# Villen-Lab/pyAscore

Hardware: AMD Instinct MI355X
Metric: PSMs/sec (Ascore.score) at 1/2/4/8 MI355X + HBM-roofline % (higher is better)
Workload: dtype f32/f64 scalar + i32 counts

## Files before the change

pyascore_amd/csrc/fused_core.hip.h:

```cpp
#ifndef PYA_FUSED_CORE_H
#define PYA_FUSED_CORE_H
#include "score_core.hip.h"
#include "localize_core.hip.h"

#define FUSED_ROUND 3

struct FusedLds {
    uint16_t *grid;
    uint4 *cum_lut;
    PeakEntry *peaks;
    float2 *resd;
    uint8_t *rkl;
    uint32_t *rec;
    float *wsl;
    float *mass_l;
    uint32_t *flag_l;
    uint8_t *site_pos;
    float *selm;
    unsigned char *sort_raw;
    PushedEntry *pushed;
    unsigned long long *site_alt;
    uint32_t *site_max, *site_tie, *n_pushed;
    float *sc;
    uint32_t *c_tr, *c_cnt;
    uint32_t *bad_tasks;
    uint32_t *t_lo, *t_off;
    float *srt_v;
    uint8_t *srt_h;
    int32_t *c_depth;
    uint32_t *c_site;
};

__host__ __device__ static inline size_t fused_align16(size_t v) { return (v + 15) & ~(size_t)15; }
__host__ __device__ static inline size_t fused_sort_bytes(uint32_t n) {
    if (n <= 64) return ((size_t)n * 10 + 15) & ~(size_t)15;
    return (((size_t)n * 6 + 15) & ~(size_t)15) + ((size_t)n / 64 + 2) * 16 + 2 * 128 * 2;
}
__host__ __device__ static inline uint32_t fused_site_cap(uint32_t push_cap) {
    const uint32_t v = (push_cap + 3u) & ~3u;
    return v > 64u ? 64u : (v < 4u ? 4u : v);
}
__host__ __device__ static inline size_t fused_post_bytes(uint32_t n_cap, uint32_t push_cap, uint32_t ent_cap, uint32_t ndir,
                                                          bool multi_z) {
    return fused_align16(fused_sort_bytes(n_cap)) + (size_t)push_cap * 16 + (size_t)fused_site_cap(push_cap) * 16 + 16 +
           (size_t)(1 + FUSED_ROUND) * 40 + (size_t)FUSED_ROUND * (16 * ndir + 4 + 4) + 16 + 64 +
           (multi_z ? fused_align16((size_t)FUSED_ROUND * ndir * 2 * ent_cap * 4) +
                          fused_align16((size_t)FUSED_ROUND * ndir * 2 * ent_cap)
                    : 0);
}
__host__ __device__ static inline size_t fused_walk_bytes(uint32_t cap) {
    return 16 * 16 + ((size_t)cap + PYA_TABLE_PAD) * 8;
}
__host__ __device__ static inline size_t fused_kept_bytes(uint32_t n_cap, uint32_t stride, uint32_t pos_cap, uint32_t ent_cap,
                                                          uint32_t ndir) {
    return fused_align16(((size_t)pos_cap + 1) * 8) + fused_align16((size_t)ent_cap * stride) + (size_t)n_cap * 16 + 256 +
           fused_align16((size_t)pos_cap + 1) + (size_t)(1 + FUSED_ROUND) * ndir * ent_cap * 4;
}
__host__ __device__ static inline size_t fused_lds_bytes(uint32_t cap, uint32_t n_cap, uint32_t stride, uint32_t pos_cap,
                                                         uint32_t ent_cap, uint32_t push_cap, uint32_t ndir, bool multi_z) {
    const size_t walk = fused_walk_bytes(cap), post = fused_post_bytes(n_cap, push_cap, ent_cap, ndir, multi_z);
    return PYA_GRID_CELLS * 2 + fused_align16(walk > post ? walk : post) +
           fused_kept_bytes(n_cap, stride, pos_cap, ent_cap, ndir) + 16;
}

DEV FusedLds fused_carve(unsigned char *raw, uint32_t cap, uint32_t n_cap, uint32_t stride, uint32_t pos_cap,
                         uint32_t ent_cap, uint32_t push_cap, uint32_t ndir, bool multi_z) {
    FusedLds f;
    f.grid = (uint16_t *)raw;
    size_t o = PYA_GRID_CELLS * 2;
    f.cum_lut = (uint4 *)(raw + o);
    f.peaks = (PeakEntry *)(raw + o + 16 * 16);
    f.sort_raw = raw + o;
    size_t q = o + fused_align16(fused_sort_bytes(n_cap));
    f.pushed = (PushedEntry *)(raw + q);
    q += (size_t)push_cap * sizeof(PushedEntry);
    const size_t sc = fused_site_cap(push_cap);
    f.site_alt = (unsigned long long *)(raw + q);
    q += sc * 8;
    f.site_max = (uint32_t *)(raw + q);
    q += sc * 4;
    f.site_tie = (uint32_t *)(raw + q);
    q += sc * 4;
    f.n_pushed = (uint32_t *)(raw + q);
    q += 16;
    f.sc = (float *)(raw + q);
    q += (size_t)(1 + FUSED_ROUND) * 40;
    f.c_tr = (uint32_t *)(raw + q);
    q += (size_t)FUSED_ROUND * ndir * 8;
    f.c_cnt = (uint32_t *)(raw + q);
    q += (size_t)FUSED_ROUND * ndir * 8;
    f.c_depth = (int32_t *)(raw + q);
    q += FUSED_ROUND * 4;
    f.c_site = (uint32_t *)(raw + q);
    q += FUSED_ROUND * 4;
    f.bad_tasks = (uint32_t *)(raw + q);
    q += 16;
    f.t_lo = (uint32_t *)(raw + q);
    f.t_off = f.t_lo + 8;
    q += 64;
    f.srt_v = (float *)(raw + q);
    q += fused_align16((size_t)FUSED_ROUND * ndir * 2 * ent_cap * 4);
    f.srt_h = (uint8_t *)(raw + q);
    const size_t walk = fused_walk_bytes(cap), post = fused_post_bytes(n_cap, push_cap, ent_cap, ndir, multi_z);
    o += fused_align16(walk > post ? walk : post);
    f.resd = (float2 *)(raw + o);
    o += fused_align16(((size_t)pos_cap + 1) * 8);
    f.rkl = (uint8_t *)(raw + o);
    o += fused_align16((size_t)ent_cap * stride);
    f.rec = (uint32_t *)(raw + o);
    o += (size_t)n_cap * 12;
    f.wsl = (float *)(raw + o);
    o += (size_t)n_cap * 4;
    f.mass_l = (float *)(raw + o);
    f.flag_l = (uint32_t *)(raw + o + 128);
    f.site_pos = (uint8_t *)(raw + o + 256);
    f.selm = (float *)(raw + o + 256 + fused_align16((size_t)pos_cap + 1));
    return f;
}


template <bool BZ>
DEV void walk_record_steps(const float2 *&rp, int rstride, StepBits &bits, float &running, const uint4 *lut, CumCounts &cum,
                           const PeakTable &tab, int zmax, double A, double B, uint8_t *&ro, int stride, int count) {
    for (int i = 0; i < count; i++, rp += rstride) {
        const float2 mm = *rp;
        running = (bits.next() ? mm.y : mm.x) + running;
        const double m = BZ ? (double)running + A : ((double)running + A) - B;
        for (int z = 1; z <= zmax; z++, ro += stride) {
            const Look k = look4(tab, charge_mz(m, z));
            int rk = k.best;
            if (k.more()) rk = look_rest(tab, k);
            cum.add(lut[rk]);
            *ro = (uint8_t)rk;
        }
    }
}
DEV CumCounts walk_record(const float2 *resd, const uint4 *lut, const PeakTable &tab, int L, int zmax, uint64_t resmask, int dir,
                          double A, double B, bool all_b_zero, uint8_t *rkl, int stride, int w) {
    const uint64_t tmask = dir ? (__brevll(resmask) >> (64 - L)) : resmask;
    const float2 *rp = resd + (dir ? L - 1 : 0);
    const int rstride = dir ? -1 : 1;
    uint8_t *ro = rkl + w;
    float running = 0.f;
    CumCounts cum = {0u, 0u, 0u};
    if (tab.half_check) {
        const uint32_t tlo = (uint32_t)tmask, thi = (uint32_t)(tmask >> 32);
        for (int step = 0; step + 1 < L; step++, rp += rstride) {
            const float2 mm = *rp;
            const uint32_t word = step < 32 ? tlo : thi;
            const bool mod = (word >> (step & 31)) & 1u;
            running = (mod ? mm.y : mm.x) + running;
            const double m = ((double)running + A) - B;
            for (int z = 1; z <= zmax; z++, ro += stride) {
                const int rk = match_rank_lds(tab, charge_mz(m, z));
                cum.add(lut[rk]);
                *ro = (uint8_t)rk;
            }
        }
        return cum;
    }
    const uint64_t M = msb_first_from(tmask, 0);
    const int n = L - 1;
    for (int seg = 0; seg < 2; seg++) {
        StepBits bits = {seg ? (uint32_t)M : (uint32_t)(M >> 32)};
        int c = (n < seg * 32 + 32 ? n : seg * 32 + 32) - seg * 32;
        if (c < 0) c = 0;
        if (all_b_zero) walk_record_steps<true>(rp, rstride, bits, running, lut, cum, tab, zmax, A, B, ro, stride, c);
        else walk_record_steps<false>(rp, rstride, bits, running, lut, cum, tab, zmax, A, B, ro, stride, c);
    }
    return cum;
}

DEV void walk_mz_only(const float2 *resd, int L, int zmax, uint64_t resmask, int dir, double A, double B, float *out) {
    const uint64_t tmask = dir ? (__brevll(resmask) >> (64 - L)) : resmask;
    const uint64_t M = msb_first_from(tmask, 0);
    const float2 *rp = resd + (dir ? L - 1 : 0);
    const int rstride = dir ? -1 : 1;
    const int Lm1 = L - 1;
    float running = 0.f;
    int step = 0;
    for (int seg = 0; seg < 2; seg++) {
        StepBits bits = {seg ? (uint32_t)M : (uint32_t)(M >> 32)};
        const int end = Lm1 < seg * 32 + 32 ? Lm1 : seg * 32 + 32;
        for (; step < end; step++, rp += rstride) {
            const float2 mm = *rp;
            running = (bits.next() ? mm.y : mm.x) + running;
            const double m = ((double)running + A) - B;
            out[step] = (float)(m + 1.007825);
            for (int z = 2; z <= zmax; z++) out[(z - 1) * Lm1 + step] = charge_mz(m, z);
        }
    }
}

DEV void walk_sums_only(const float2 *resd, int L, uint64_t resmask, int dir, float *out) {
    const uint64_t tmask = dir ? (__brevll(resmask) >> (64 - L)) : resmask;
    const uint64_t M = msb_first_from(tmask, 0);
    const float2 *rp = resd + (dir ? L - 1 : 0);
    const int rstride = dir ? -1 : 1;
    const int Lm1 = L - 1;
    float running = 0.f;
    int step = 0;
    for (int seg = 0; seg < 2; seg++) {
        StepBits bits = {seg ? (uint32_t)M : (uint32_t)(M >> 32)};
        const int end = Lm1 < seg * 32 + 32 ? Lm1 : seg * 32 + 32;
        for (; step < end; step++, rp += rstride) {
            const float2 mm = *rp;
            running = (bits.next() ? mm.y : mm.x) + running;
            out[step] = running;
        }
    }
}

DEV int partners_in_run(const float *run, int n, int p2, float me, int side, float err) {
    int j = 0;
    for (int step = p2 >> 1; step > 0; step >>= 1) {
        const int probe = j + step;
        const float o = probe - 1 < n ? run[probe - 1] : __builtin_huge_valf();
        const float dd = side ? (o - me) : (me - o);
        if (side ? (dd <= -err) : (dd >= err)) j = probe;
    }
    int cnt = 0;
    for (int q = j; q < j + 2 && q < n; q++) {
        const float dd = side ? (run[q] - me) : (me - run[q]);
        cnt += (__builtin_fabsf(dd) < err) ? 1 : 0;
    }
    return cnt;
}

#define FUSED_LOCAL_CHUNKS 8
struct LocalTable {
    const float *mz;
    const uint8_t *rank;
    int R, status;
};

template <bool BOTH, bool ZM, bool WIDE = false>
DEV bool fused_body(const BatchDev &b, uint32_t psm, unsigned char *lds_raw, uint32_t cap, uint32_t n_cap, uint32_t stride,
                    uint32_t pos_cap, uint32_t ent_cap, uint32_t push_cap, const LocalTable *local = nullptr) {
    const int lane = lane_id();
    const DevConfig *cfg = b.cfg;
    const int ndir = BOTH ? 2 : 1;
    const FusedLds f = fused_carve(lds_raw, cap, n_cap, stride, pos_cap, ent_cap, push_cap, (uint32_t)ndir, ZM);
    STAMP_BEGIN();
    STAMP_T(b, 38, false);
    float lmz[FUSED_LOCAL_CHUNKS];
    uint32_t lrk[FUSED_LOCAL_CHUNKS];
    if (local) {
#pragma unroll
        for (int q = 0; q < FUSED_LOCAL_CHUNKS; q++) {
            const int i = q * 64 + lane_id();
            lmz[q] = i < local->R ? local->mz[i] : __builtin_huge_valf();
            lrk[q] = i < local->R ? (uint32_t)local->rank[i] : (uint32_t)PYA_NO_MATCH;
        }
        wave_lds_sync();
    }
    if (lane < 32) {
        f.mass_l[lane] = cfg->res_mass[lane];
        f.flag_l[lane] = cfg->res_modifiable[lane];
    }
    const uint64_t *dw = b.desc + (size_t)psm * PYA_DESC_WORDS;
    const int64_t p0 = (int64_t)dw[0], pep0 = (int64_t)dw[1], s0 = (int64_t)dw[2], a0 = (int64_t)dw[3];
    const uint64_t w4 = dw[4], w5 = dw[5];
    const int L = (int)(w4 & 0xffffu), n_aux = (int)((w4 >> 16) & 0xffffu), k = (int)((w4 >> 32) & 0xffffu);
    const int zmax = ZM ? (int)(w4 >> 56) : 1;
    const int N = (int)(uint32_t)w5;
    const uint64_t *order = b.order_tab + (uint32_t)(w5 >> 32);
    const int status = local ? local->status : b.status[psm];
    const int R = local ? local->R : (int)b.ret_n[psm];

    const uint32_t max_k = b.max_k;
    float *out_asc = b.ascores + (size_t)psm * max_k;
    uint64_t *out_alt = b.alt_mask + (size_t)psm * max_k;
    for (uint32_t a = lane; a < max_k; a += 64) {
        out_asc[a] = 0.f;
        out_alt[a] = 0ull;
    }
    if (status != PYA_ST_OK) {
        if (lane == 0) {
            b.best_score[psm] = -1.f;
            b.best_sig[psm] = 0ull;
            b.n_sig_out[psm] = -1;
        }
        return false;
    }
    STAMP_T(b, 39, false);
    const bool two_pass = BOTH && WIDE && N > 32;
    const int s = (BOTH && !two_pass) ? (lane & 31) : lane;
    const int dir = BOTH ? (two_pass ? 0 : (lane >> 5)) : (cfg->n_fwd > 0 ? 0 : 1);
    const bool active = s < N;
    const uint32_t letter = lane < L ? (uint32_t)b.pep[pep0 + lane] : (uint32_t)'A';
    const uint64_t bits = active ? order[s] : 0ull;
    uint32_t aux_pos = 0;
    float aux_mass = 0.f;
    if (lane < n_aux) {
        aux_pos = b.aux_pos[a0 + lane];
        aux_mass = b.aux_mass[a0 + lane];
    }
    if (local) {
#pragma unroll
        for (int q = 0; q < FUSED_LOCAL_CHUNKS; q++) {
            const int i = q * 64 + lane;
            if (i < R + PYA_TABLE_PAD) {
                PeakEntry e;
                e.mz = lmz[q];
                e.rank = lrk[q];
                f.peaks[i] = e;
            }
        }
    } else {
        copy_peak_table(b.ret + p0, R, f.peaks, lane, 64);
    }
    PeakTable tab;
    tab.e = f.peaks;
    tab.g_cell = nullptr;
    tab.g_e = b.ret + p0;
    tab.n = R;
    tab.err = cfg->mz_error;
    tab.half_check = cfg->mz_error > 0.49f;
    double Af = 0., Bf = 0., Ab = 0., Bb = 0.;
    if (cfg->n_fwd > 0) type_constants(cfg->types[0], &Af, &Bf);
    if (cfg->n_fwd < cfg->n_types) type_constants(cfg->types[cfg->n_fwd], &Ab, &Bb);
    wave_lds_sync();
    STAMP_T(b, 48, false);
    float m0, m1;
    uint64_t site_mask;
    {
        const bool in = lane < L;
        const uint32_t li = (letter - 'A') & 31u;
        m0 = f.mass_l[li];
        const bool modifiable = in && ((f.flag_l[li] & 1u) || (cfg->allow_n && lane == 0) || (cfg->allow_c && lane == L - 1));
        m1 = m0 + cfg->mod_mass;
        for (int base = 0; base < n_aux; base += 64) {
            const int n = n_aux - base < 64 ? n_aux - base : 64;
            if (base > 0) {
                aux_pos = 0;
                aux_mass = 0.f;
                if (lane < n) {
                    aux_pos = b.aux_pos[a0 + base + lane];
                    aux_mass = b.aux_mass[a0 + base + lane];
                }
            }
            for (int j = 0; j < n; j++) {
                const uint32_t pos = (uint32_t)__builtin_amdgcn_readlane((int)aux_pos, j);
                const float am = __int_as_float(__builtin_amdgcn_readlane(__float_as_int(aux_mass), j));
                const int idx = pos > 0 ? (int)pos - 1 : 0;
                if (idx == lane) {
                    m0 += am;
                    m1 += am;
                }
            }
        }
        site_mask = __ballot(modifiable);
        if (in) f.resd[lane] = make_float2(m0, m1);
        if (modifiable) f.site_pos[mask_rank(site_mask)] = (uint8_t)lane;
    }
    STAMP_T(b, 49, false);
    grid_build(&tab, f.grid);
    STAMP_T(b, 50, false);
    if (lane < 16) f.cum_lut[lane] = fused_cum_entry((uint32_t)lane);
    const int Lm1 = L - 1;
    const uint64_t resmask = deposit_sites(bits, site_mask);
    const int w = !active ? (int)stride - 1 : (BOTH ? dir * N + s : s);
    const bool presorted = !__any(lane < L && !(m0 > 0.f && m1 > 0.f));
    const float wide_min = 2.f * cfg->mz_error + 0.02f;
    const bool wide = !__any(lane < L && !(m0 > wide_min && m1 > wide_min));
    wave_lds_sync();
    STAMP_T(b, 40, false);
    CumCounts cum = walk_record(f.resd, f.cum_lut, tab, L, zmax, resmask, dir, dir ? Ab : Af, dir ? Bb : Bf, Bf == 0. && Bb == 0.,
                                f.rkl, (int)stride, w);
    if (two_pass) {
        const CumCounts back = walk_record(f.resd, f.cum_lut, tab, L, zmax, resmask, 1, Ab, Bb, Bf == 0. && Bb == 0., f.rkl, (int)stride,
                                           active ? N + s : (int)stride - 1);
        cum.a += back.a;
        cum.b += back.b;
        cum.c += back.c;
    } else if (BOTH) {
        uint32_t *r3 = f.rec + (size_t)s * 3;
        if (active && lane >= 32) {
            r3[0] = cum.a;
            r3[1] = cum.b;
            r3[2] = cum.c;
        }
        wave_lds_sync();
        if (active && lane < 32) {
            cum.a += r3[0];
            cum.b += r3[1];
            cum.c += r3[2];
        }
    }
    wave_lds_sync();
    STAMP_T(b, 41, false);

    const uint32_t nfrag = (uint32_t)ndir * (uint32_t)Lm1 * (uint32_t)zmax;
    int fail = 0;
    float ws = 0.f;
// ... 437 lines not shown
```

pyascore_amd/csrc/host_internal.h:

```cpp
#ifndef PYA_HOST_INTERNAL_H
#define PYA_HOST_INTERNAL_H
#include <hip/hip_runtime_api.h>

#include <algorithm>
#include <atomic>
#include <cmath>
#include <cstdarg>
#include <cstddef>
#include <cstdio>
#include <cstdlib>
#include <chrono>
#include <cstring>
#include <condition_variable>
#include <map>
#include <memory>
#include <mutex>
#include <string>
#include <thread>
#include <unordered_map>
#include <vector>

#include "../../include/pyascore_hip.h"
#include "common.h"

void pya_score_table_extend(float mz_error, uint32_t n_top, uint32_t n_to, std::vector<float> &lut,
                            std::vector<uint32_t> &off);
extern "C" {
size_t pya_bin_lds_bytes(uint32_t cap);
size_t pya_score_lds_bytes(uint32_t cap, uint32_t prefix, uint32_t with_nl, uint32_t compact);
size_t pya_localize_lds_bytes(uint32_t push_cap, uint32_t n_cap, uint32_t pos_cap, uint32_t pool_cap, uint32_t sb);
int pya_launch_bin(const BatchDev *b, const uint32_t *d_ids, uint32_t n_ids, uint32_t cap, uint32_t types, hipStream_t stream);
int pya_launch_bin_select(const BatchDev *b, const uint32_t *d_ids, uint32_t n_ids, uint32_t scap, uint32_t types, hipStream_t stream);
size_t pya_bin_select_lds_bytes(uint32_t scap);
int pya_launch_bin_exact(const BatchDev *b, uint32_t n_total, uint32_t cap, uint32_t types, hipStream_t stream);
int pya_launch_fan_out(const uint32_t *d_spec_of, const uint32_t *d_spec_ret_n, const int32_t *d_spec_status, uint32_t *d_ret_n,
                       int32_t *d_status, uint32_t n_psm, hipStream_t stream);
int pya_launch_score(const BatchDev *b, const uint32_t *d_ids, uint32_t n_ids, uint32_t cap, uint32_t prefix,
                     uint32_t with_nl, uint32_t compact, uint32_t node_cap, uint32_t node_cols, uint32_t node_words,
                     uint32_t res_cap, uint32_t nl_cap, hipStream_t stream);
size_t pya_score_node_lds_bytes(uint32_t cap, uint32_t with_nl, uint32_t node_cap, uint32_t node_cols, uint32_t node_words,
                                uint32_t res_cap, uint32_t nl_cap);
int pya_launch_localize(const BatchDev *b, const uint32_t *d_ids, uint32_t n_ids, uint32_t push_cap,
                        uint32_t n_cap, uint32_t pos_cap, uint32_t pool_cap, uint32_t sb, uint32_t gtp,
                        uint32_t plain, uint32_t sort_room, hipStream_t stream);
size_t pya_tiny_lds_bytes(uint32_t cap, uint32_t prefix, uint32_t with_nl, uint32_t compact, uint32_t push_cap,
                          uint32_t n_cap, uint32_t pos_cap, uint32_t pool_cap, uint32_t sb);
int pya_launch_tiny(const BatchDev *b, uint32_t n_psm, uint32_t cap, uint32_t prefix, uint32_t with_nl,
                    uint32_t compact, uint32_t push_cap, uint32_t n_cap, uint32_t pos_cap, uint32_t pool_cap,
                    uint32_t sb, uint32_t gtp, hipStream_t stream);
size_t pya_one_lds_bytes(uint32_t cap, uint32_t prefix, uint32_t with_nl, uint32_t compact, uint32_t push_cap, uint32_t n_cap,
                         uint32_t pos_cap, uint32_t pool_cap, uint32_t sb, uint32_t use_fused, uint32_t f_n_cap, uint32_t f_stride,
                         uint32_t f_ent_cap, uint32_t f_push_cap, uint32_t multi_z);
int pya_launch_one(const BatchDev *b, const OneMeta *m, uint32_t cap, uint32_t prefix, uint32_t with_nl, uint32_t compact,
                   uint32_t push_cap, uint32_t n_cap, uint32_t pos_cap, uint32_t pool_cap, uint32_t sb, uint32_t gtp,
                   uint32_t use_fused, uint32_t f_n_cap, uint32_t f_stride, uint32_t f_ent_cap, uint32_t f_push_cap,
                   uint32_t multi_z, int32_t *host_status, uint32_t *host_flag, hipStream_t stream);
int pya_launch_ambiguity(const BatchDev *b, uint32_t psm, uint32_t peak_cap, uint32_t list_cap,
                         uint64_t ref_bits, uint64_t oth_bits, const float *d_scores, float ref_ws,
                         float oth_ws, float *d_out, hipStream_t stream);
int pya_launch_debug_sort(const float *d_keys, uint32_t n, uint32_t *d_perm, hipStream_t stream);
int pya_launch_pack_records(const float *best_score, const int32_t *n_sig, const uint64_t *best_sig, const float *ascores,
                            const uint64_t *alt_mask, uint32_t k, uint32_t res_k, uint64_t n_psm, int32_t *out, hipStream_t stream);
int pya_launch_debug_wave_ops(const int32_t *d_in, int32_t *d_out, hipStream_t stream);
size_t pya_score_big_lds_bytes(uint32_t cap, uint32_t pos_cap, uint32_t kc);
int pya_launch_score_big(const BatchDev *b, const uint32_t *d_ids, uint32_t n_ids, uint32_t cap, uint32_t pos_cap, uint32_t kc,
                         uint32_t inline_on, hipStream_t stream);
size_t pya_localize_recount_lds_bytes(uint32_t cap, uint32_t push_cap, uint32_t pos_cap, uint32_t pool_cap, uint32_t sb);
size_t pya_localize_hash_lds_bytes(uint32_t push_cap, uint32_t n_cap, uint32_t pos_cap, uint32_t sb, uint32_t vc, uint32_t hs,
                                   uint32_t pp, uint32_t max_k, uint32_t n_nl);
int pya_launch_localize_hash(const BatchDev *b, const uint32_t *d_ids, uint32_t n_ids, uint32_t push_cap, uint32_t n_cap,
                             uint32_t pos_cap, uint32_t pool_cap, uint32_t sb, uint32_t gtp, uint32_t vc, uint32_t hs, uint32_t pp,
                             uint32_t n_nl, hipStream_t stream);
int pya_launch_localize_recount(const BatchDev *b, const uint32_t *d_ids, uint32_t n_ids, uint32_t cap, uint32_t push_cap,
                                uint32_t pos_cap, uint32_t pool_cap, uint32_t sb, uint32_t gtp, uint32_t *d_redo_count, uint32_t *d_redo_ids, hipStream_t stream);
int pya_launch_score_big_list(const BatchDev *b, const uint32_t *d_count, const uint32_t *d_ids, uint32_t n_max, uint32_t cap,
                              uint32_t pos_cap, uint32_t kc, hipStream_t stream);
uint32_t pya_big_inline_max(void);
size_t pya_fused_lds_bytes(uint32_t cap, uint32_t n_cap, uint32_t stride, uint32_t pos_cap, uint32_t ent_cap, uint32_t push_cap,
                           uint32_t both, uint32_t multi_z);
int pya_launch_fused(const BatchDev *b, const uint32_t *d_ids, uint32_t n_ids, uint32_t cap, uint32_t n_cap,
                     uint32_t stride, uint32_t pos_cap, uint32_t ent_cap, uint32_t push_cap, uint32_t both,
                     uint32_t multi_z, uint32_t *d_redo_count, uint32_t *d_redo_ids, hipStream_t stream);
size_t pya_score_cnt_lds_bytes(uint32_t cap, uint32_t pos_cap, uint32_t kc, uint32_t k_cap, uint32_t n_cap);
int pya_launch_score_cnt(const BatchDev *b, const uint32_t *d_ids, uint32_t n_ids, uint32_t cap, uint32_t pos_cap, uint32_t kc, uint32_t k_cap,
                         uint32_t n_cap, hipStream_t stream);
size_t pya_score_cntg_lds_bytes(uint32_t cap, uint32_t pos_cap, uint32_t k_cap, uint32_t n_cap, uint32_t nl_cap);
int pya_launch_score_cntg(const BatchDev *b, const uint32_t *d_ids, uint32_t n_ids, uint32_t cap, uint32_t pos_cap, uint32_t k_cap, uint32_t n_cap,
                          uint32_t nl_cap, hipStream_t stream);
size_t pya_bin_global_scratch_bytes(uint32_t cap);
int pya_launch_bin_global(const BatchDev *b, const uint32_t *d_ids, uint32_t n_ids, unsigned char *d_scratch, uint64_t stride,
                          uint32_t cap, uint32_t types, hipStream_t stream);
size_t pya_general_lds_bytes(uint32_t l_cap, uint32_t list_cap);
size_t pya_general_scratch_bytes(uint32_t n_cap, uint32_t push_cap);
int pya_launch_general(const BatchDev *b, const uint32_t *d_ids, uint32_t n_ids, unsigned char *d_scratch, const uint64_t *d_scratch_off,
                       uint32_t l_cap, uint32_t list_cap, hipStream_t stream);
int pya_launch_general_ambiguity(const BatchDev *b, uint32_t psm, uint32_t l_cap, uint32_t list_cap, uint64_t ref_bits,
                                 uint64_t oth_bits, const float *d_scores, uint32_t n_scores, float ref_ws, float oth_ws,
                                 float *d_out, hipStream_t stream);
size_t pya_evidence_lds_bytes(uint32_t l_cap, uint32_t list_cap);
int pya_launch_evidence(const BatchDev *b, const uint32_t *d_ids, uint32_t n_ids, void *d_out, uint32_t l_cap, uint32_t list_cap,
                        hipStream_t stream);
size_t pya_ions_lds_bytes(uint32_t l_cap, uint32_t list_cap);
uint32_t pya_ions_scan_tiles(uint32_t n);
int pya_launch_ions(const BatchDev *b, const uint32_t *d_ids, uint32_t n_ids, const void *d_evid, int64_t *d_off, void *d_out, uint64_t cap,
                    uint32_t *d_over, uint32_t l_cap, uint32_t list_cap, hipStream_t stream);
int pya_launch_ions_scan(int64_t *d_off, uint32_t n, uint64_t *d_tiles, hipStream_t stream);
size_t pya_named_lds_bytes(uint32_t l_cap, uint32_t list_cap);
int pya_launch_named(const BatchDev *b, const uint32_t *d_ids, uint32_t n_ids, const int64_t *d_q_off, const uint64_t *d_q_bits,
                     uint64_t n_q, void *d_out, int32_t *d_counts, float *d_scores, uint32_t *d_over, uint32_t l_cap,
                     uint32_t list_cap, hipStream_t stream);
size_t pya_sites_lds_bytes(uint32_t l_cap, uint32_t list_cap);
int pya_launch_sites(const BatchDev *b, const uint32_t *d_ids, uint32_t n_ids, const int64_t *d_site_off, uint64_t n_out,
                     uint32_t sig_cap, void *d_out, uint32_t l_cap, hipStream_t stream);
size_t pya_probs_lds_bytes(uint32_t l_cap, const PcCaps *caps, uint32_t sw);
size_t pya_probs_cnt_bytes(const PcCaps *caps);
int pya_launch_probs(const BatchDev *b, const uint32_t *d_ids, uint32_t n_ids, const int64_t *d_site_off, uint64_t n_out,
                     uint32_t sig_cap, void *d_out, void *d_psms, uint32_t l_cap, const PcCaps *caps, uint32_t sw, hipStream_t stream);
size_t pya_ranked_lds_bytes(uint32_t l_cap, const PcCaps *caps, uint32_t sw);
int pya_launch_ranked(const BatchDev *b, const uint32_t *d_ids, uint32_t n_ids, const int64_t *d_site_off, uint32_t top_k,
                      uint32_t sig_cap, void *d_out, uint32_t l_cap, const PcCaps *caps, uint32_t sw, hipStream_t stream);
int pya_launch_rollup_clear(void *d_table, uint64_t n_slots, hipStream_t stream);
int pya_launch_rollup(const int64_t *d_site_off, uint64_t n_psm, uint64_t n_rec, const void *d_site_probs, const void *d_psm_probs,
                      const int32_t *d_slot, uint64_t n_slots, double threshold, const uint32_t *d_psm_id, uint32_t psm_base,
                      const uint64_t *best_sig, const float *ascores, uint32_t max_k, void *d_table, uint32_t *d_over, uint32_t grid[2],
                      hipStream_t stream);
size_t pya_mz_profile_lds_bytes(uint32_t l_cap);
int pya_launch_mz_profile(const BatchDev *b, const uint32_t *d_ids, uint32_t n_ids, const int32_t *d_run, uint64_t n_slots,
                          const pya_mz_profile_params *prm, void *d_table, uint32_t *d_over, uint32_t l_cap, hipStream_t stream);
int pya_launch_mz_fit(const void *d_table, uint64_t n_slots, double inv_ppm, uint32_t min_ions, void *d_cal, hipStream_t stream);
int pya_launch_mz_apply(const void *d_mz, uint32_t mz_type, const int64_t *d_peak_off, uint64_t n_spectra, const int32_t *d_run,
                        const void *d_cal, uint64_t n_slots, double inv_band, void *d_out, uint32_t *d_over, hipStream_t stream);
uint64_t pya_flr_layout_bytes(uint64_t n_slots);
int pya_launch_flr(const void *d_table, uint64_t n_slots, const uint8_t *d_cls, uint32_t reported_only, void *d_work, void *d_out,
                   uint32_t *d_order, uint32_t *d_n_ranked, hipEvent_t *phase, hipStream_t stream);
uint64_t pya_pform_layout_bytes(uint64_t n_entries);
int pya_launch_pform(const int64_t *d_site_off, uint64_t n_psm, const void *d_site_probs, const void *d_psm_probs, const int32_t *d_group,
                     double threshold, const uint32_t *d_psm_id, uint32_t psm_base, const uint64_t *best_sig, const float *ascores, uint32_t max_k,
                     const void *d_src0, uint64_t n0, const void *d_src1, uint64_t n1, void *d_work, void *d_out, uint64_t cap, uint32_t *d_n,
                     hipEvent_t *phase, hipStream_t stream);
int pya_launch_localize_redo(const BatchDev *b, const uint32_t *d_count, const uint32_t *d_ids, uint32_t n_max,
                             uint32_t push_cap, uint32_t n_cap, uint32_t pos_cap, uint32_t pool_cap, uint32_t sb,
                             uint32_t gtp, hipStream_t stream);
}



const size_t kMaxLds = 160 * 1024;
const uint32_t kBucketLimits[] = {64, 512, 4096, PYA_FAST_SIGNATURES};
const int kNumBuckets = 4;
const size_t kRedoHead = 64;
const size_t kStageLimit = 1u << 20;

template <typename T>
struct DevBuf {
    T *p = nullptr;
    size_t n = 0;
    bool owned = true;
    DevBuf() {}
    DevBuf(const DevBuf &) = delete;
    DevBuf &operator=(const DevBuf &) = delete;
    ~DevBuf() { release(); }
    void release() {
        if (p && owned) (void)hipFree(p);
        p = nullptr;
        n = 0;
        owned = true;
    }
    void adopt(void *ptr, size_t count) {
        release();
        p = (T *)ptr;
        n = count;
        owned = false;
    }
    hipError_t fill(const T *src, hipStream_t s = nullptr) {
        if (n == 0 || !src) return hipSuccess;
        return hipMemcpyAsync(p, src, n * sizeof(T), hipMemcpyHostToDevice, s);
    }
    hipError_t alloc(size_t count) {
        release();
        n = count;
        if (count == 0) count = 1;
        return hipMalloc((void **)&p, count * sizeof(T));
    }
    hipError_t upload(const T *src, size_t count, hipStream_t s = nullptr) {
        hipError_t e = alloc(count);
        if (e != hipSuccess || count == 0) return e;
        return hipMemcpyAsync(p, src, count * sizeof(T), hipMemcpyHostToDevice, s);
    }
    size_t bytes() const { return n * sizeof(T); }
    bool take_if_fits(DevBuf &other, size_t count) {
        if (!other.p || !other.owned || other.n < count) return false;
        release();
        p = other.p;
        n = other.n;
        other.p = nullptr;
        other.n = 0;
        return true;
    }
    void give_to(DevBuf &other) {
        if (!p || !owned) return;
        if (other.p && other.n >= n) return;
        other.release();
        other.p = p;
        other.n = n;
        p = nullptr;
        n = 0;
    }
};

inline uint64_t binom(uint32_t n, uint32_t k) {
    if (k > n) return 0;
    if (k > n - k) k = n - k;
    unsigned __int128 r = 1;
    for (uint32_t i = 1; i <= k; i++) {
        r = r * (n - k + i) / i;
        if (r > (unsigned __int128)1 << 62) return ~0ull;
    }
    return (uint64_t)r;
}

uint32_t next_pow2(uint32_t v);

inline bool is_forward(char t) { return t == 'b' || t == 'c'; }
inline bool is_backward(char t) { return t == 'y' || t == 'z' || t == 'Z'; }

inline float std_residue_mass(char c) {
    switch (c) {
        case 'G': return 57.02146f;   case 'A': return 71.03711f;   case 'S': return 87.03203f;
        case 'P': return 97.05276f;   case 'V': return 99.06841f;   case 'T': return 101.04768f;
        case 'C': return 103.00919f;  case 'L': return 113.08406f;  case 'I': return 113.08406f;
        case 'N': return 114.04293f;  case 'D': return 115.02694f;  case 'Q': return 128.05858f;
        case 'K': return 128.09496f;  case 'E': return 129.04259f;  case 'M': return 131.04049f;
// ... 608 lines not shown
```

pyascore_amd/csrc/score_localize.hip:

```cpp
#include "fused_core.hip.h"

#ifndef FUSED_WAVES
#define FUSED_WAVES 6
#endif

template <bool BOTH, bool ZM, bool WIDE = false>
__global__ __launch_bounds__(64, FUSED_WAVES) void pya_score_localize_kernel(
    BatchDev b, const uint32_t *psm_ids, uint32_t n_ids, uint32_t cap, uint32_t n_cap, uint32_t stride, uint32_t pos_cap,
    uint32_t ent_cap, uint32_t push_cap, uint32_t *redo_count, uint32_t *redo_ids) {
    extern __shared__ __attribute__((aligned(16))) unsigned char lds_raw[];
    if (blockIdx.x >= n_ids) return;
    const uint32_t psm = psm_ids[xcd_slot(blockIdx.x, n_ids)];
    const bool declined = fused_body<BOTH, ZM, WIDE>(b, psm, lds_raw, cap, n_cap, stride, pos_cap, ent_cap, push_cap);
    if (declined && lane_id() == 0) redo_ids[atomicAdd(redo_count, 1u)] = psm;
}

extern "C" size_t pya_fused_lds_bytes(uint32_t cap, uint32_t n_cap, uint32_t stride, uint32_t pos_cap, uint32_t ent_cap,
                                      uint32_t push_cap, uint32_t both, uint32_t multi_z) {
    return fused_lds_bytes(cap, n_cap, stride, pos_cap, ent_cap, push_cap, both ? 2u : 1u, multi_z != 0);
}

extern "C" int pya_launch_fused(const BatchDev *b, const uint32_t *d_ids, uint32_t n_ids, uint32_t cap, uint32_t n_cap,
                                uint32_t stride, uint32_t pos_cap, uint32_t ent_cap, uint32_t push_cap, uint32_t both,
                                uint32_t multi_z, uint32_t *d_redo_count, uint32_t *d_redo_ids, hipStream_t stream) {
    if (n_ids == 0) return 0;
    const size_t lds = fused_lds_bytes(cap, n_cap, stride, pos_cap, ent_cap, push_cap, both ? 2u : 1u, multi_z != 0);
#define PYA_FUSED_LAUNCH(B, Z, W)                                                                                          \
    do {                                                                                                                   \
        hipError_t e = PYA_ENSURE_MAX_LDS((pya_score_localize_kernel<B, Z, W>));                                           \
        if (e != hipSuccess) return (int)e;                                                                                \
        hipLaunchKernelGGL((pya_score_localize_kernel<B, Z, W>), dim3(n_ids), dim3(64), lds, stream, *b, d_ids, n_ids, cap, \
                           n_cap, stride, pos_cap, ent_cap, push_cap, d_redo_count, d_redo_ids);                           \
    } while (0)
    const bool wide = both && n_cap > 32u;
    if (both && multi_z && wide) PYA_FUSED_LAUNCH(true, true, true);
    else if (both && wide) PYA_FUSED_LAUNCH(true, false, true);
    else if (both && multi_z) PYA_FUSED_LAUNCH(true, true, false);
    else if (both) PYA_FUSED_LAUNCH(true, false, false);
    else if (multi_z) PYA_FUSED_LAUNCH(false, true, false);
    else PYA_FUSED_LAUNCH(false, false, false);
#undef PYA_FUSED_LAUNCH
    return (int)hipGetLastError();
}
```

Baseline: 205.3 million.

## Add liveness-aware compact LDS layout and higher-occupancy kernel variant

Replaces the hand-carved LDS layout with a table-driven layout that records each region's live phases. A compact form overlaps the post-phase selection buffer with walk-phase space and packs the mass/flag tables into the rkl/rec region. When the compact footprint is small enough, a FULL variant launches with launch_bounds of 8 waves instead of 6. The aim is to cut LDS per block so more workgroups fit per CU. The risk is aliasing bugs if liveness assumptions are wrong, plus register pressure from the tighter launch bound.

```diff
diff --git a/pyascore_amd/csrc/fused_core.hip.h b/pyascore_amd/csrc/fused_core.hip.h
--- a/pyascore_amd/csrc/fused_core.hip.h
+++ b/pyascore_amd/csrc/fused_core.hip.h
@@ -40,81 +40,139 @@
     const uint32_t v = (push_cap + 3u) & ~3u;
     return v > 64u ? 64u : (v < 4u ? 4u : v);
 }
-__host__ __device__ static inline size_t fused_post_bytes(uint32_t n_cap, uint32_t push_cap, uint32_t ent_cap, uint32_t ndir,
-                                                          bool multi_z) {
-    return fused_align16(fused_sort_bytes(n_cap)) + (size_t)push_cap * 16 + (size_t)fused_site_cap(push_cap) * 16 + 16 +
-           (size_t)(1 + FUSED_ROUND) * 40 + (size_t)FUSED_ROUND * (16 * ndir + 4 + 4) + 16 + 64 +
-           (multi_z ? fused_align16((size_t)FUSED_ROUND * ndir * 2 * ent_cap * 4) +
-                          fused_align16((size_t)FUSED_ROUND * ndir * 2 * ent_cap)
-                    : 0);
-}
-__host__ __device__ static inline size_t fused_walk_bytes(uint32_t cap) {
-    return 16 * 16 + ((size_t)cap + PYA_TABLE_PAD) * 8;
-}
-__host__ __device__ static inline size_t fused_kept_bytes(uint32_t n_cap, uint32_t stride, uint32_t pos_cap, uint32_t ent_cap,
-                                                          uint32_t ndir) {
-    return fused_align16(((size_t)pos_cap + 1) * 8) + fused_align16((size_t)ent_cap * stride) + (size_t)n_cap * 16 + 256 +
-           fused_align16((size_t)pos_cap + 1) + (size_t)(1 + FUSED_ROUND) * ndir * ent_cap * 4;
+
+enum {
+    FL_GRID, FL_CUM_LUT, FL_PEAKS,
+    FL_SORT_RAW, FL_PUSHED, FL_SITE_ALT, FL_SITE_MAX, FL_SITE_TIE, FL_N_PUSHED, FL_SC, FL_C_TR, FL_C_CNT, FL_C_DEPTH, FL_C_SITE,
+    FL_BAD_TASKS, FL_T_LO, FL_T_OFF, FL_SRT_V, FL_SRT_H, FL_SELM,
+    FL_RESD, FL_RKL, FL_REC, FL_WSL, FL_MASS_L, FL_FLAG_L, FL_SITE_POS,
+    FL_COUNT
+};
+enum { FP_INPUTS, FP_WALK, FP_POST, FP_HANDOVER };
+
+struct FusedLayout {
+    size_t off[FL_COUNT], size[FL_COUNT];
+    uint8_t from[FL_COUNT], to[FL_COUNT];
+    size_t total;
+};
+
+__host__ __device__ static inline FusedLayout fused_lds_layout_form(uint32_t cap, uint32_t n_cap, uint32_t stride, uint32_t pos_cap,
+                                                                     uint32_t ent_cap, uint32_t push_cap, uint32_t ndir, bool multi_z,
+                                                                     bool compact) {
+    FusedLayout y;
+    size_t o = 0;
+#define FL_PUT(a, bytes, step, f, t)                                                                                       \
+    do {                                                                                                                   \
+        y.off[a] = o;                                                                                                      \
+        y.size[a] = (size_t)(bytes);                                                                                       \
+        y.from[a] = (f);                                                                                                   \
+        y.to[a] = (t);                                                                                                     \
+        o += (step);                                                                                                       \
+    } while (0)
+    FL_PUT(FL_GRID, PYA_GRID_CELLS * 2, PYA_GRID_CELLS * 2, FP_INPUTS, FP_HANDOVER);
+    const size_t base = o;
+    FL_PUT(FL_CUM_LUT, 16 * 16, 16 * 16, FP_INPUTS, FP_WALK);
+    FL_PUT(FL_PEAKS, ((size_t)cap + PYA_TABLE_PAD) * 8, ((size_t)cap + PYA_TABLE_PAD) * 8, FP_INPUTS, FP_WALK);
+    const size_t walk_end = o;
+    o = base;
+    const size_t sc = fused_site_cap(push_cap), tasks = (size_t)FUSED_ROUND * ndir;
+    FL_PUT(FL_SORT_RAW, fused_sort_bytes(n_cap), fused_align16(fused_sort_bytes(n_cap)), FP_POST, FP_POST);
+    FL_PUT(FL_PUSHED, (size_t)push_cap * 16, (size_t)push_cap * 16, FP_POST, FP_POST);
+    FL_PUT(FL_SITE_ALT, sc * 8, sc * 8, FP_POST, FP_POST);
+    FL_PUT(FL_SITE_MAX, sc * 4, sc * 4, FP_POST, FP_POST);
+    FL_PUT(FL_SITE_TIE, sc * 4, sc * 4, FP_POST, FP_POST);
+    FL_PUT(FL_N_PUSHED, 4, 16, FP_POST, FP_POST);
+    FL_PUT(FL_SC, (size_t)(1 + FUSED_ROUND) * 40, (size_t)(1 + FUSED_ROUND) * 40, FP_POST, FP_POST);
+    FL_PUT(FL_C_TR, tasks * 8, tasks * 8, FP_POST, FP_POST);
+    FL_PUT(FL_C_CNT, tasks * 8, tasks * 8, FP_POST, FP_POST);
+    FL_PUT(FL_C_DEPTH, FUSED_ROUND * 4, FUSED_ROUND * 4, FP_POST, FP_POST);
+    FL_PUT(FL_C_SITE, FUSED_ROUND * 4, FUSED_ROUND * 4, FP_POST, FP_POST);
+    FL_PUT(FL_BAD_TASKS, 4, 16, FP_POST, FP_POST);
+    FL_PUT(FL_T_LO, 32, 32, FP_POST, FP_POST);
+    FL_PUT(FL_T_OFF, 32, 32, FP_POST, FP_POST);
+    const size_t srt = multi_z ? tasks * 2 * ent_cap : 0;
+    FL_PUT(FL_SRT_V, srt * 4, fused_align16(srt * 4), FP_POST, FP_POST);
+    FL_PUT(FL_SRT_H, srt, fused_align16(srt), FP_POST, FP_POST);
+    const size_t selm = (size_t)(1 + FUSED_ROUND) * ndir * ent_cap * 4;
+    if (compact) {
+        o = fused_align16(o);
+        FL_PUT(FL_SELM, selm, selm, FP_POST, FP_POST);
+    }
+    o = fused_align16(o > walk_end ? o : walk_end);
+    FL_PUT(FL_RESD, ((size_t)pos_cap + 1) * 8, fused_align16(((size_t)pos_cap + 1) * 8), FP_INPUTS, FP_POST);
+    const size_t shared = o;
+    FL_PUT(FL_RKL, (size_t)ent_cap * stride, fused_align16((size_t)ent_cap * stride), FP_WALK, FP_POST);
+    FL_PUT(FL_REC, (size_t)n_cap * 12, (size_t)n_cap * 12, FP_WALK, FP_HANDOVER);
+    FL_PUT(FL_WSL, (size_t)n_cap * 4, (size_t)n_cap * 4, FP_WALK, FP_HANDOVER);
+    const size_t shared_end = o > shared + 256 ? o : shared + 256;
+    if (compact) o = shared;
+    FL_PUT(FL_MASS_L, 128, 128, FP_INPUTS, FP_INPUTS);
+    FL_PUT(FL_FLAG_L, 128, 128, FP_INPUTS, FP_INPUTS);
+    if (compact) o = shared_end;
+    FL_PUT(FL_SITE_POS, (size_t)pos_cap + 1, fused_align16((size_t)pos_cap + 1), FP_INPUTS, FP_POST);
+    if (!compact) FL_PUT(FL_SELM, selm, selm, FP_POST, FP_POST);
+#undef FL_PUT
+    y.total = o + 16;
+    return y;
+}
+#ifndef FUSED_FULL_LDS_MAX
+#define FUSED_FULL_LDS_MAX 5632u
+#endif
+__host__ __device__ static inline uint32_t fused_lds_per_cu(size_t bytes) {
+    const size_t n = (size_t)160 * 1024 / ((bytes + 511) & ~(size_t)511);
+    return n > 32 ? 32u : (uint32_t)n;
+}
+__host__ __device__ static inline bool fused_lds_full(uint32_t cap, uint32_t n_cap, uint32_t stride, uint32_t pos_cap,
+                                                      uint32_t ent_cap, uint32_t push_cap, uint32_t ndir, bool multi_z) {
+    return !multi_z && fused_lds_layout_form(cap, n_cap, stride, pos_cap, ent_cap, push_cap, ndir, multi_z, true).total <= FUSED_FULL_LDS_MAX;
+}
+__host__ __device__ static inline bool fused_lds_compact(uint32_t cap, uint32_t n_cap, uint32_t stride, uint32_t pos_cap,
+                                                         uint32_t ent_cap, uint32_t push_cap, uint32_t ndir, bool multi_z) {
+    if (fused_lds_full(cap, n_cap, stride, pos_cap, ent_cap, push_cap, ndir, multi_z)) return true;
+    return fused_lds_per_cu(fused_lds_layout_form(cap, n_cap, stride, pos_cap, ent_cap, push_cap, ndir, multi_z, true).total) >
+           fused_lds_per_cu(fused_lds_layout_form(cap, n_cap, stride, pos_cap, ent_cap, push_cap, ndir, multi_z, false).total);
+}
+__host__ __device__ static inline FusedLayout fused_lds_layout(uint32_t cap, uint32_t n_cap, uint32_t stride, uint32_t pos_cap,
+                                                                uint32_t ent_cap, uint32_t push_cap, uint32_t ndir, bool multi_z) {
+    return fused_lds_layout_form(cap, n_cap, stride, pos_cap, ent_cap, push_cap, ndir, multi_z,
+                                 fused_lds_compact(cap, n_cap, stride, pos_cap, ent_cap, push_cap, ndir, multi_z));
 }
 __host__ __device__ static inline size_t fused_lds_bytes(uint32_t cap, uint32_t n_cap, uint32_t stride, uint32_t pos_cap,
                                                          uint32_t ent_cap, uint32_t push_cap, uint32_t ndir, bool multi_z) {
-    const size_t walk = fused_walk_bytes(cap), post = fused_post_bytes(n_cap, push_cap, ent_cap, ndir, multi_z);
-    return PYA_GRID_CELLS * 2 + fused_align16(walk > post ? walk : post) +
-           fused_kept_bytes(n_cap, stride, pos_cap, ent_cap, ndir) + 16;
+    return fused_lds_layout(cap, n_cap, stride, pos_cap, ent_cap, push_cap, ndir, multi_z).total;
 }
 
 DEV FusedLds fused_carve(unsigned char *raw, uint32_t cap, uint32_t n_cap, uint32_t stride, uint32_t pos_cap,
-                         uint32_t ent_cap, uint32_t push_cap, uint32_t ndir, bool multi_z) {
+                         uint32_t ent_cap, uint32_t push_cap, uint32_t ndir, bool multi_z, bool compact) {
+    const FusedLayout y = fused_lds_layout_form(cap, n_cap, stride, pos_cap, ent_cap, push_cap, ndir, multi_z, compact);
     FusedLds f;
-    f.grid = (uint16_t *)raw;
-    size_t o = PYA_GRID_CELLS * 2;
-    f.cum_lut = (uint4 *)(raw + o);
-    f.peaks = (PeakEntry *)(raw + o + 16 * 16);
-    f.sort_raw = raw + o;
-    size_t q = o + fused_align16(fused_sort_bytes(n_cap));
-    f.pushed = (PushedEntry *)(raw + q);
-    q += (size_t)push_cap * sizeof(PushedEntry);
-    const size_t sc = fused_site_cap(push_cap);
-    f.site_alt = (unsigned long long *)(raw + q);
-    q += sc * 8;
-    f.site_max = (uint32_t *)(raw + q);
-    q += sc * 4;
-    f.site_tie = (uint32_t *)(raw + q);
-    q += sc * 4;
-    f.n_pushed = (uint32_t *)(raw + q);
-    q += 16;
-    f.sc = (float *)(raw + q);
-    q += (size_t)(1 + FUSED_ROUND) * 40;
-    f.c_tr = (uint32_t *)(raw + q);
-    q += (size_t)FUSED_ROUND * ndir * 8;
-    f.c_cnt = (uint32_t *)(raw + q);
-    q += (size_t)FUSED_ROUND * ndir * 8;
-    f.c_depth = (int32_t *)(raw + q);
-    q += FUSED_ROUND * 4;
-    f.c_site = (uint32_t *)(raw + q);
-    q += FUSED_ROUND * 4;
-    f.bad_tasks = (uint32_t *)(raw + q);
-    q += 16;
-    f.t_lo = (uint32_t *)(raw + q);
-    f.t_off = f.t_lo + 8;
-    q += 64;
-    f.srt_v = (float *)(raw + q);
-    q += fused_align16((size_t)FUSED_ROUND * ndir * 2 * ent_cap * 4);
-    f.srt_h = (uint8_t *)(raw + q);
-    const size_t walk = fused_walk_bytes(cap), post = fused_post_bytes(n_cap, push_cap, ent_cap, ndir, multi_z);
-    o += fused_align16(walk > post ? walk : post);
-    f.resd = (float2 *)(raw + o);
-    o += fused_align16(((size_t)pos_cap + 1) * 8);
-    f.rkl = (uint8_t *)(raw + o);
-    o += fused_align16((size_t)ent_cap * stride);
-    f.rec = (uint32_t *)(raw + o);
-    o += (size_t)n_cap * 12;
-    f.wsl = (float *)(raw + o);
-    o += (size_t)n_cap * 4;
-    f.mass_l = (float *)(raw + o);
-    f.flag_l = (uint32_t *)(raw + o + 128);
-    f.site_pos = (uint8_t *)(raw + o + 256);
-    f.selm = (float *)(raw + o + 256 + fused_align16((size_t)pos_cap + 1));
+    f.grid = (uint16_t *)(raw + y.off[FL_GRID]);
+    f.cum_lut = (uint4 *)(raw + y.off[FL_CUM_LUT]);
+    f.peaks = (PeakEntry *)(raw + y.off[FL_PEAKS]);
+    f.sort_raw = raw + y.off[FL_SORT_RAW];
+    f.pushed = (PushedEntry *)(raw + y.off[FL_PUSHED]);
+    f.site_alt = (unsigned long long *)(raw + y.off[FL_SITE_ALT]);
+    f.site_max = (uint32_t *)(raw + y.off[FL_SITE_MAX]);
+    f.site_tie = (uint32_t *)(raw + y.off[FL_SITE_TIE]);
+    f.n_pushed = (uint32_t *)(raw + y.off[FL_N_PUSHED]);
+    f.sc = (float *)(raw + y.off[FL_SC]);
+    f.c_tr = (uint32_t *)(raw + y.off[FL_C_TR]);
+    f.c_cnt = (uint32_t *)(raw + y.off[FL_C_CNT]);
+    f.c_depth = (int32_t *)(raw + y.off[FL_C_DEPTH]);
+    f.c_site = (uint32_t *)(raw + y.off[FL_C_SITE]);
+    f.bad_tasks = (uint32_t *)(raw + y.off[FL_BAD_TASKS]);
+    f.t_lo = (uint32_t *)(raw + y.off[FL_T_LO]);
+    f.t_off = (uint32_t *)(raw + y.off[FL_T_OFF]);
+    f.srt_v = (float *)(raw + y.off[FL_SRT_V]);
+    f.srt_h = (uint8_t *)(raw + y.off[FL_SRT_H]);
+    f.selm = (float *)(raw + y.off[FL_SELM]);
+    f.resd = (float2 *)(raw + y.off[FL_RESD]);
+    f.rkl = (uint8_t *)(raw + y.off[FL_RKL]);
+    f.rec = (uint32_t *)(raw + y.off[FL_REC]);
+    f.wsl = (float *)(raw + y.off[FL_WSL]);
+    f.mass_l = (float *)(raw + y.off[FL_MASS_L]);
+    f.flag_l = (uint32_t *)(raw + y.off[FL_FLAG_L]);
+    f.site_pos = (uint8_t *)(raw + y.off[FL_SITE_POS]);
     return f;
 }
 
@@ -234,13 +292,14 @@
     int R, status;
 };
 
-template <bool BOTH, bool ZM, bool WIDE = false>
+template <bool BOTH, bool ZM, bool WIDE = false, int COMPACT = -1>
 DEV bool fused_body(const BatchDev &b, uint32_t psm, unsigned char *lds_raw, uint32_t cap, uint32_t n_cap, uint32_t stride,
                     uint32_t pos_cap, uint32_t ent_cap, uint32_t push_cap, const LocalTable *local = nullptr) {
     const int lane = lane_id();
     const DevConfig *cfg = b.cfg;
     const int ndir = BOTH ? 2 : 1;
-    const FusedLds f = fused_carve(lds_raw, cap, n_cap, stride, pos_cap, ent_cap, push_cap, (uint32_t)ndir, ZM);
+    const bool compact = COMPACT >= 0 ? COMPACT != 0 : fused_lds_compact(cap, n_cap, stride, pos_cap, ent_cap, push_cap, (uint32_t)ndir, ZM);
+    const FusedLds f = fused_carve(lds_raw, cap, n_cap, stride, pos_cap, ent_cap, push_cap, (uint32_t)ndir, ZM, compact);
     STAMP_BEGIN();
     STAMP_T(b, 38, false);
     float lmz[FUSED_LOCAL_CHUNKS];
diff --git a/pyascore_amd/csrc/host_internal.h b/pyascore_amd/csrc/host_internal.h
--- a/pyascore_amd/csrc/host_internal.h
+++ b/pyascore_amd/csrc/host_internal.h
@@ -78,6 +78,9 @@
 uint32_t pya_big_inline_max(void);
 size_t pya_fused_lds_bytes(uint32_t cap, uint32_t n_cap, uint32_t stride, uint32_t pos_cap, uint32_t ent_cap, uint32_t push_cap,
                            uint32_t both, uint32_t multi_z);
+uint32_t pya_fused_lds_layout(uint32_t cap, uint32_t n_cap, uint32_t stride, uint32_t pos_cap, uint32_t ent_cap, uint32_t push_cap,
+                              uint32_t both, uint32_t multi_z, uint32_t *offsets, uint32_t *sizes, uint32_t *live_from,
+                              uint32_t *live_to);
 int pya_launch_fused(const BatchDev *b, const uint32_t *d_ids, uint32_t n_ids, uint32_t cap, uint32_t n_cap,
                      uint32_t stride, uint32_t pos_cap, uint32_t ent_cap, uint32_t push_cap, uint32_t both,
                      uint32_t multi_z, uint32_t *d_redo_count, uint32_t *d_redo_ids, hipStream_t stream);
diff --git a/pyascore_amd/csrc/score_localize.hip b/pyascore_amd/csrc/score_localize.hip
--- a/pyascore_amd/csrc/score_localize.hip
+++ b/pyascore_amd/csrc/score_localize.hip
@@ -3,15 +3,16 @@
 #ifndef FUSED_WAVES
 #define FUSED_WAVES 6
 #endif
+#define FUSED_WAVES_FULL 8
 
-template <bool BOTH, bool ZM, bool WIDE = false>
-__global__ __launch_bounds__(64, FUSED_WAVES) void pya_score_localize_kernel(
+template <bool BOTH, bool ZM, bool WIDE = false, bool FULL = false, bool COMPACT = false>
+__global__ __launch_bounds__(64, FULL ? FUSED_WAVES_FULL : FUSED_WAVES) void pya_score_localize_kernel(
     BatchDev b, const uint32_t *psm_ids, uint32_t n_ids, uint32_t cap, uint32_t n_cap, uint32_t stride, uint32_t pos_cap,
     uint32_t ent_cap, uint32_t push_cap, uint32_t *redo_count, uint32_t *redo_ids) {
     extern __shared__ __attribute__((aligned(16))) unsigned char lds_raw[];
     if (blockIdx.x >= n_ids) return;
     const uint32_t psm = psm_ids[xcd_slot(blockIdx.x, n_ids)];
-    const bool declined = fused_body<BOTH, ZM, WIDE>(b, psm, lds_raw, cap, n_cap, stride, pos_cap, ent_cap, push_cap);
+    const bool declined = fused_body<BOTH, ZM, WIDE, COMPACT ? 1 : 0>(b, psm, lds_raw, cap, n_cap, stride, pos_cap, ent_cap, push_cap);
     if (declined && lane_id() == 0) redo_ids[atomicAdd(redo_count, 1u)] = psm;
 }
 
@@ -20,25 +21,53 @@
     return fused_lds_bytes(cap, n_cap, stride, pos_cap, ent_cap, push_cap, both ? 2u : 1u, multi_z != 0);
 }
 
+extern "C" uint32_t pya_fused_lds_layout(uint32_t cap, uint32_t n_cap, uint32_t stride, uint32_t pos_cap, uint32_t ent_cap,
+                                         uint32_t push_cap, uint32_t both, uint32_t multi_z, uint32_t *offsets, uint32_t *sizes,
+                                         uint32_t *live_from, uint32_t *live_to) {
+    const FusedLayout y = fused_lds_layout(cap, n_cap, stride, pos_cap, ent_cap, push_cap, both ? 2u : 1u, multi_z != 0);
+    for (int a = 0; a < FL_COUNT; a++) {
+        if (offsets) offsets[a] = (uint32_t)y.off[a];
+        if (sizes) sizes[a] = (uint32_t)y.size[a];
+        if (live_from) live_from[a] = y.from[a];
+        if (live_to) live_to[a] = y.to[a];
+    }
+    return FL_COUNT;
+}
+
 extern "C" int pya_launch_fused(const BatchDev *b, const uint32_t *d_ids, uint32_t n_ids, uint32_t cap, uint32_t n_cap,
                                 uint32_t stride, uint32_t pos_cap, uint32_t ent_cap, uint32_t push_cap, uint32_t both,
                                 uint32_t multi_z, uint32_t *d_redo_count, uint32_t *d_redo_ids, hipStream_t stream) {
     if (n_ids == 0) return 0;
     const size_t lds = fused_lds_bytes(cap, n_cap, stride, pos_cap, ent_cap, push_cap, both ? 2u : 1u, multi_z != 0);
-#define PYA_FUSED_LAUNCH(B, Z, W)                                                                                          \
+#define PYA_FUSED_LAUNCH(B, Z, W, F, C)                                                                                    \
     do {                                                                                                                   \
-        hipError_t e = PYA_ENSURE_MAX_LDS((pya_score_localize_kernel<B, Z, W>));                                           \
+        hipError_t e = PYA_ENSURE_MAX_LDS((pya_score_localize_kernel<B, Z, W, F, C>));                                     \
         if (e != hipSuccess) return (int)e;                                                                                \
-        hipLaunchKernelGGL((pya_score_localize_kernel<B, Z, W>), dim3(n_ids), dim3(64), lds, stream, *b, d_ids, n_ids, cap, \
-                           n_cap, stride, pos_cap, ent_cap, push_cap, d_redo_count, d_redo_ids);                           \
+        hipLaunchKernelGGL((pya_score_localize_kernel<B, Z, W, F, C>), dim3(n_ids), dim3(64), lds, stream, *b, d_ids,      \
+                           n_ids, cap, n_cap, stride, pos_cap, ent_cap, push_cap, d_redo_count, d_redo_ids);               \
+    } while (0)
+#define PYA_FUSED_FORM_Z1(B, W)                                                                                            \
+    do {                                                                                                                   \
+        if (full) PYA_FUSED_LAUNCH(B, false, W, true, true);                                                               \
+        else if (compact) PYA_FUSED_LAUNCH(B, false, W, false, true);                                                      \
+        else PYA_FUSED_LAUNCH(B, false, W, false, false);                                                                  \
+    } while (0)
+#define PYA_FUSED_FORM_ZM(B, W)                                                                                            \
+    do {                                                                                                                   \
+        if (compact) PYA_FUSED_LAUNCH(B, true, W, false, true);                                                            \
+        else PYA_FUSED_LAUNCH(B, true, W, false, false);                                                                   \
     } while (0)
     const bool wide = both && n_cap > 32u;
-    if (both && multi_z && wide) PYA_FUSED_LAUNCH(true, true, true);
-    else if (both && wide) PYA_FUSED_LAUNCH(true, false, true);
-    else if (both && multi_z) PYA_FUSED_LAUNCH(true, true, false);
-    else if (both) PYA_FUSED_LAUNCH(true, false, false);
-    else if (multi_z) PYA_FUSED_LAUNCH(false, true, false);
-    else PYA_FUSED_LAUNCH(false, false, false);
+    const bool full = fused_lds_full(cap, n_cap, stride, pos_cap, ent_cap, push_cap, both ? 2u : 1u, multi_z != 0);
+    const bool compact = fused_lds_compact(cap, n_cap, stride, pos_cap, ent_cap, push_cap, both ? 2u : 1u, multi_z != 0);
+    if (both && multi_z && wide) PYA_FUSED_FORM_ZM(true, true);
+    else if (both && wide) PYA_FUSED_FORM_Z1(true, true);
+    else if (both && multi_z) PYA_FUSED_FORM_ZM(true, false);
+    else if (both) PYA_FUSED_FORM_Z1(true, false);
+    else if (multi_z) PYA_FUSED_FORM_ZM(false, false);
+    else PYA_FUSED_FORM_Z1(false, false);
+#undef PYA_FUSED_FORM_ZM
+#undef PYA_FUSED_FORM_Z1
 #undef PYA_FUSED_LAUNCH
     return (int)hipGetLastError();
 }
```

New measurement: 216.4 million (median of 6 runs). 1.05x the previous value.
